# facebookresearch/vggsfm

Measured on AMD Instinct MI355X. Metric: BA LM-iterations/sec, higher is better.
Workload: dtype f64

## Files before the change

### vggsfm_amd/ba.py

```python
import copy
import ctypes
from dataclasses import dataclass
from typing import Optional

import math
import os

import numpy as np
import torch

from . import _lib
from .ba_options import LOSS_ID, TERMINATION, BundleAdjustmentOptions

MODEL_ID = {"SIMPLE_PINHOLE": 0, "SIMPLE_RADIAL": 1}
GROUP = 16
CHUNK = 1024
SUB = 32
MIN_CHUNK = 128
OVERLAP_FACTORIZATION = False
OVERLAP_MIN_OBS, OVERLAP_MIN_FRAMES = 1_000_000, 8 * GROUP
TILE_BATCHES = 3
CHOL_CUS = 32


# ... 664 lines not shown
                             camera_type, options, False, constant_points=constant, constant_pose_frames=[0],
                             filter_negative_depth=False)


def _c_options(options: BundleAdjustmentOptions, overlap=True):
    so = options.solver_options
    return _lib.BAOptions(so.max_num_iterations, so.max_num_consecutive_invalid_steps, int(so.jacobi_scaling),
                          so.function_tolerance, so.gradient_tolerance, so.parameter_tolerance,
                          so.initial_trust_region_radius, so.max_trust_region_radius, so.min_trust_region_radius,
                          so.min_lm_diagonal, so.max_lm_diagonal, so.min_relative_decrease,
                          CHOL_CUS if (overlap and OVERLAP_FACTORIZATION) else 0)


def _summary_dict(summ, log, n):
    its = [dict(iteration=l.iteration, cost=l.cost, cost_change=l.cost_change, gradient_max_norm=l.gradient_max_norm,
                step_norm=l.step_norm, relative_decrease=l.relative_decrease, radius=l.radius,
                successful=bool(l.successful)) for l in log[:n]]
    return dict(initial_cost=summ.initial_cost, final_cost=summ.final_cost, num_iterations=summ.num_iterations,
                num_successful_steps=summ.num_successful_steps, num_unsuccessful_steps=summ.num_unsuccessful_steps,
                termination=summ.termination, termination_str=TERMINATION.get(summ.termination, "?"),
                n_reduced=summ.n_reduced, iterations=its)


def solve(problem: DeviceProblem, options: Optional[BundleAdjustmentOptions] = None, workspace=None):
    L = _lib.lib()
    glue = _hook("VGGSFM_LEGACY_GLUE")
    if glue is not None:
        L.vgg_ba_set_tile_rhs(2 | (4 if glue == "1" else 0))
    options = options or BundleAdjustmentOptions()
    problem.refine_focal = options.refine_focal_length
    problem.refine_extra = options.refine_extra_params
    problem.loss = LOSS_ID[options.loss_function_type]
    problem.loss_scale = options.loss_function_scale
    cp = problem.c_struct()
    co = _c_options(options)
    nbytes = L.vgg_ba_workspace_bytes(ctypes.byref(cp), ctypes.byref(co))
    if workspace is None or workspace.numel() < nbytes:
        workspace = torch.empty(nbytes, dtype=torch.uint8, device=problem.pts.device)
    summ = _lib.BASummary()
    cap = options.solver_options.max_num_iterations + 2
    log = (_lib.BAIteration * cap)()
    _lib.check(L.vgg_ba_solve(ctypes.byref(cp), ctypes.byref(co), workspace, workspace.numel(), ctypes.byref(summ), log, cap,
                              _lib.stream_ptr()), "vgg_ba_solve")
    out = _summary_dict(summ, log, summ.num_log)
    if options.print_summary:
        print(f"Bundle adjustment report: residuals {problem.num_obs * 2}, parameters reduced {summ.n_reduced}, "
              f"iterations {summ.num_iterations}, cost {summ.initial_cost:.6g} -> {summ.final_cost:.6g}, "
              f"{out['termination_str']}")
    return out, workspace


# ... 73 lines not shown
```

### vggsfm_amd/csrc/ba.hip

```cpp
#include <mutex>
#include <type_traits>
#include <vector>

#include "camera_model.hpp"
#include "../../include/vggsfm_amd.h"

namespace vgg {

int cholesky_solve_enqueue(double* A, double* b, int n, double* inv_blocks, int32_t* device_fail, const int32_t* skip_flag,
                           hipStream_t st, const CholOverlap* overlap, int split_a, int split_b, const int32_t* first_blk,
                           bool flags_cleared);
int32_t* cholesky_dataflow_flags(double* ws, int n, size_t* count);
size_t cholesky_workspace_bytes(int n);
void dataflow_signal(int32_t* flag, hipStream_t st);

constexpr int kGroup = 16;
#ifndef VGG_OFFDIAG_OCC
#define VGG_OFFDIAG_OCC 3
#endif
#ifndef VGG_DIAG_OCC
#define VGG_DIAG_OCC 4
#endif
#ifndef VGG_DIAG_FULL_DEPTH
#define VGG_DIAG_FULL_DEPTH 2
// ... 17 lines not shown
#define VGG_PS_OCC 2
#endif
#ifndef VGG_CP_OCC_RHS
#define VGG_CP_OCC_RHS 2
#endif
#ifndef VGG_CP_OCC
#define VGG_CP_OCC 2
#endif
#ifndef VGG_ABLATE
#define VGG_ABLATE 0
#endif
constexpr int kSub = 32;
constexpr int kMaxWG = 2048;
constexpr int kCamSplitMax = 16;
constexpr int kCamNV = 48;
constexpr int kPackPad = 1024;

struct Ctl {
  double radius, decrease_factor, x_cost, initial_cost, gmax_cams, gmax, cand_cost, mcc, step_norm, rel;
  int32_t iteration, done, termination, need_lin, scale_ready, invalid_streak, num_succ, num_unsucc;
  int32_t linear_fail, accept, rank, world, grad_logged;
  int32_t step_arrivals;
  int32_t merged_glue_launches, merged_step_sums;
};

struct Dims {
  int C, P, O, NI, model, kd, only_k, shared, BDp, n_red, kdsh, loss;
  double loss_scale;
};

constexpr int kYc = 12;
static inline size_t y_slot_doubles(const Dims& d) { return (d.shared || d.kd == 0) ? (size_t)kYc : (size_t)d.BDp * 3; }

struct Ws {
  Ctl* ctl;
  vgg_ba_iteration* log;
  double *cand_q, *cand_t, *cand_intr, *cand_pts;
  double *scale_c, *scale_p, *colsq_c, *dsq_c, *dy;
  uint8_t* active;
  double* lin;
  double *U, *g, *costc;
  double* sys;
  double *S, *rhs;
  double* S2;
  double* gmax_pts;
  double* stepsum;
// ... 19 lines not shown
  int tile_rhs;
  double* lin_cand;
  double *U_cand, *g_cand, *cost_cand;
  size_t lin_count, sys_count, total_bytes;
};

static inline size_t align_up(size_t x, size_t a) { return (x + a - 1) / a * a; }


static Dims make_dims(const vgg_ba_problem* pb) {
  Dims d;
  d.C = pb->num_cams; d.P = pb->num_pts; d.O = pb->num_obs; d.NI = pb->num_intr; d.model = pb->camera_model;
  const int rf = pb->refine_focal ? 1 : 0, rk = (pb->refine_extra && pb->camera_model == kSimpleRadial) ? 1 : 0;
  d.kd = rf + rk;
  d.only_k = (!rf && rk) ? 1 : 0;
  d.shared = (pb->num_intr == 1) ? 1 : 0;
  d.BDp = 6 + d.kd;
  d.n_red = 6 * d.C + d.kd * d.NI;
  d.kdsh = d.shared ? d.kd : 0;
  d.loss = pb->loss; d.loss_scale = pb->loss_scale;
  return d;
}

struct Tuning { int lpp, longt, cam_wgs, point_wgs, tile_rhs, legacy_glue; };
static Tuning g_tuning = {0, -1, 0, 0, 2, 0};

static Ws carve(const Dims& d, int max_iters, int num_chunks, int num_segments, void* base) {
  Ws w;
  size_t off = 0;
  auto take = [&](size_t bytes) { size_t o = off; off = align_up(off + bytes, 256); return (char*)base + o; };
  w.ctl = (Ctl*)take(sizeof(Ctl));
  w.log = (vgg_ba_iteration*)take(sizeof(vgg_ba_iteration) * (size_t)(max_iters + 2));
  w.cand_q = (double*)take(8ull * 4 * d.C); w.cand_t = (double*)take(8ull * 3 * d.C);
  w.cand_intr = (double*)take(8ull * 4 * d.NI); w.cand_pts = (double*)take(8ull * 3 * d.P);
  w.scale_c = (double*)take(8ull * d.n_red); w.scale_p = (double*)take(8ull * 3 * d.P);
  w.colsq_c = (double*)take(8ull * d.n_red); w.dsq_c = (double*)take(8ull * d.n_red);
  w.dy = (double*)take(8ull * d.n_red);
  w.active = (uint8_t*)take(d.n_red);
  w.lin_count = (size_t)d.C * d.BDp * d.BDp + (size_t)d.C * d.BDp + d.C;
  w.lin = (double*)take(8ull * w.lin_count);
  w.U = w.lin; w.g = w.U + (size_t)d.C * d.BDp * d.BDp; w.costc = w.g + (size_t)d.C * d.BDp;
  w.sys_count = (size_t)d.n_red * d.n_red + d.n_red;
  w.sys = (double*)take(8ull * w.sys_count);
  w.S = w.sys; w.rhs = w.S + (size_t)d.n_red * d.n_red;
  w.S2 = (double*)take(8ull * (size_t)d.n_red * d.n_red);
  w.packed_count = (size_t)d.n_red * (d.n_red + 1) / 2 + d.n_red;
  w.packed = (double*)take(8ull * (w.packed_count + 2 * kPackPad));
  w.pk_mine = (double*)take(8ull * (w.packed_count + 2));
// ... 126 lines not shown
  }
  return rho[0];
}

__device__ __forceinline__ double loss_rho0(const Dims& d, double s) {
  double rho[3];
  loss_eval(d.loss, d.loss_scale, s, rho);
  return rho[0];
}

template <int NV>
__device__ __forceinline__ void block_sum(double* v, double* lds , double* out ) {
  const int wave = threadIdx.x >> 6, lane = threadIdx.x & 63;
#pragma unroll
  for (int i = 0; i < NV; ++i) {
    const double s = wave_sum(v[i]);
    if (lane == 0) lds[wave * NV + i] = s;
  }
  __syncthreads();
  if (threadIdx.x < NV) out[threadIdx.x] = lds[threadIdx.x] + lds[NV + threadIdx.x] + lds[2 * NV + threadIdx.x] + lds[3 * NV + threadIdx.x];
  __syncthreads();
}

__global__ void init_kernel(DevProblem pb, Ws w, vgg_ba_options opt, int rank, int world) {
  const Dims& d = pb.d;
  const int j = blockIdx.x * blockDim.x + threadIdx.x;
  if (j == 0) {
    Ctl c;
    memset(&c, 0, sizeof(c));
    c.radius = opt.initial_trust_region_radius; c.decrease_factor = 2.0; c.need_lin = 1; c.rank = rank; c.world = world;
    *w.ctl = c;
    w.gmax_pts[0] = 0; for (int i = 0; i < 4; ++i) w.stepsum[i] = 0;
  }
  if (j < d.n_red) {
    bool act;
    if (j < 6 * d.C) {
      const int c = j / 6, k = j - 6 * c;
      const unsigned f = pb.cam_const ? pb.cam_const[c] : 0u;
      act = (pb.col_ptr[c + 1] > pb.col_ptr[c]) || world > 1;
      if (f & 1u) act = false;
      if (k >= 3 && (f & (2u << (k - 3)))) act = false;
    } else {
      const int a = (j - 6 * d.C) / d.kd;
      act = !(pb.intr_const && pb.intr_const[a]);
      if (!d.shared && world == 1 && !(pb.col_ptr[a + 1] > pb.col_ptr[a])) act = false;
    }
// ... 91 lines not shown
#pragma unroll
        for (int k = i; k < BD; ++k) acc[u++] += F[i] * F[k] + F[BD + i] * F[BD + k];
#pragma unroll
      for (int i = 0; i < BD; ++i) acc[NU + i] += F[i] * r[0] + F[BD + i] * r[1];
      acc[NU + BD] += rho0;
    } else {
      double R0[1 + KD], R1[1 + KD];
      R0[0] = r[0] - (E[0] * h0 + E[1] * h1v + E[2] * h2);
      R1[0] = r[1] - (E[3] * h0 + E[4] * h1v + E[5] * h2);
#pragma unroll
      for (int m = 0; m < KD; ++m) {
        if (m < kdsh) {
          const double* M = Mc + 3 * m;
          R0[1 + m] = -(E[0] * M[0] + E[1] * M[1] + E[2] * M[2]);
          R1[1 + m] = -(E[3] * M[0] + E[4] * M[1] + E[5] * M[2]);
        } else { R0[1 + m] = 0; R1[1 + m] = 0; }
      }
#pragma unroll
      for (int i = 0; i < BD; ++i)
#pragma unroll
        for (int m = 0; m < 1 + KD; ++m) acc[i * (1 + KD) + m] += F[i] * R0[m] + F[BD + i] * R1[m];
    }
  }
  block_sum<NV>(acc, red, tot);
  static_assert(NV <= kCamNV, "cam_split row");
  if (threadIdx.x < NV) w.cam_split[((size_t)c * kCamSplitMax + blockIdx.y) * kCamNV + threadIdx.x] = tot[threadIdx.x];
}

template <bool BYPASS>
__device__ __forceinline__ void reduce_step_body(const Ws& w, int nparts, int C, double (*red)[256]) {
  auto ld = [](const double* p) -> double {
    return BYPASS ? __hip_atomic_load(p, __ATOMIC_RELAXED, __HIP_MEMORY_SCOPE_AGENT) : *p;
  };
  double s[4] = {0, 0, 0, 0};
  for (int i = threadIdx.x; i < C; i += 256) s[0] += ld(w.cost_cand + i);
  for (int i = threadIdx.x; i < nparts; i += 256)
    for (int k = 1; k < 4; ++k) s[k] += ld(w.part_F + 4 * i + k);
  for (int k = 0; k < 4; ++k) red[k][threadIdx.x] = s[k];
  __syncthreads();
  for (int st = 128; st > 0; st >>= 1) {
    if (threadIdx.x < st) for (int k = 0; k < 4; ++k) red[k][threadIdx.x] += red[k][threadIdx.x + st];
    __syncthreads();
  }
  if (threadIdx.x < 4) w.stepsum[threadIdx.x] = red[threadIdx.x][0];
}

template <int KD, int MODE>
// ... 1394 lines not shown
  for (; ch + 1 < c1; ch += 2) { s0 += src[(size_t)ch * R * R]; s1 += src[(size_t)(ch + 1) * R * R]; }
  if (ch < c1) s0 += src[(size_t)ch * R * R];
  const int hi = ri > cj ? ri : cj, lo = ri > cj ? cj : ri;
  double v = -(s0 + s1);
  if constexpr (BD == 6) {
    const double mi = w.active[ri] ? w.scale_c[ri] : 0.0, mj = w.active[cj] ? w.scale_c[cj] : 0.0;
    v *= mi * mj;
  }
  if (gI == gJ && a == b) {
    const double* U = w.U + (size_t)ca * UBD * UBD;
    double t = 0.0;
    if (global_terms) t = w.scale_c[ri] * w.scale_c[cj] * U[i * UBD + j];
    if (ri == cj) {
      const double dsq = lm_damping(U[i * UBD + i], w.scale_c[ri], radius, opt);
      w.dsq_c[ri] = dsq;
      if (global_terms) t += dsq;
    }
    v = v + t;
  }
  w.S[(size_t)hi * n + lo] = v;
}

template <int KD>
__global__ void cam_update_kernel(DevProblem pb, Ws w) {
  if (w.ctl->done) return;
  const Dims& d = pb.d;
  const int c = blockIdx.x * blockDim.x + threadIdx.x;
  if (c > d.C) return;
  double step = 0, xn = 0;
  if (c < d.C) {
    double dl[6];
    for (int k = 0; k < 6; ++k) {
      const int j = 6 * c + k;
      const double dyv = w.active[j] ? w.scale_c[j] * w.rhs[j] : 0.0;
      w.dy[j] = dyv;
      dl[k] = -dyv;
    }
    double qn[4];
    quat_plus(pb.cam_q + 4 * c, dl, qn);
    const bool pose_var = !(pb.cam_const && (pb.cam_const[c] & 1u));
    for (int k = 0; k < 4; ++k) { w.cand_q[4 * c + k] = qn[k]; const double df = qn[k] - pb.cam_q[4 * c + k]; step += df * df; if (pose_var) xn += pb.cam_q[4 * c + k] * pb.cam_q[4 * c + k]; }
    for (int k = 0; k < 3; ++k) { const double tn = pb.cam_t[3 * c + k] + dl[3 + k]; w.cand_t[3 * c + k] = tn; step += dl[3 + k] * dl[3 + k]; if (pose_var) xn += pb.cam_t[3 * c + k] * pb.cam_t[3 * c + k]; }
  }
  const int a = d.shared ? ((c == d.C) ? 0 : -1) : ((c < d.C) ? c : -1);
  if (a >= 0) {
    double in4[4];
    for (int k = 0; k < 4; ++k) in4[k] = pb.intr[4 * a + k];
    for (int k = 0; k < KD; ++k) {
      const int j = 6 * d.C + KD * a + k;
      const double dyv = w.active[j] ? w.scale_c[j] * w.rhs[j] : 0.0;
      w.dy[j] = dyv;
      const int slot = (KD == 2) ? (k == 0 ? 0 : 3) : (d.only_k ? 3 : 0);
      in4[slot] -= dyv;
      step += dyv * dyv;
    }
    const bool intr_var = KD > 0 && !(pb.intr_const && pb.intr_const[a]);
    const int np = (d.model == kSimpleRadial) ? 4 : 3;
    for (int k = 0; k < 4; ++k) { w.cand_intr[4 * a + k] = in4[k]; if (intr_var && k < np) xn += pb.intr[4 * a + k] * pb.intr[4 * a + k]; }
  }
  w.cam_part[3 * c] = step;
  w.cam_part[3 * c + 1] = xn;
  w.cam_part[3 * c + 2] = 0.0;
}

template <int KD, bool LDSCAM, int LPP, bool LONGT = false>
__global__ __launch_bounds__(256, VGG_PS_OCC) void point_step_kernel(DevProblem pb, Ws w) {
  constexpr int BD = 6 + KD;
  __shared__ double red[4][3];
  extern __shared__ double cam_cache[];
  if (w.ctl->done) return;
  const Dims& d = pb.d;
  constexpr int PPW = 64 / LPP;
  const int wave = threadIdx.x >> 6, lane = threadIdx.x & 63;
  const int sub = lane / LPP, sl = lane % LPP;
  const int nw = gridDim.x * 4 * PPW;
  double s_mcc = 0, s_step = 0, s_xn = 0;
  const double* lq = cam_cache;
  const double* lt = lq + 9 * d.C;
  const double* ldy = lt + 3 * d.C;
  const double* lfl = ldy + 6 * d.C;
  if (LDSCAM) {
    double* cc = cam_cache;
    for (int i = threadIdx.x; i < d.C; i += 256) {
      quat_to_R(pb.cam_q + 4 * i, cc + 9 * i);
      cc[18 * d.C + i] = pb.cam_const ? (double)pb.cam_const[i] : 0.0;
    }
    for (int i = threadIdx.x; i < 3 * d.C; i += 256) cc[9 * d.C + i] = pb.cam_t[i];
    for (int i = threadIdx.x; i < 6 * d.C; i += 256) cc[(ldy - cam_cache) + i] = w.dy[i];
    __syncthreads();
  }
  (void)lfl;
  int p = (blockIdx.x * 4 + wave) * PPW + sub;
  constexpr int NPF = LONGT ? 4 : 2;
  int n_o0 = 0, n_o1 = 0;
  ObsPf<NPF> n_pf;
  double n_X0 = 0, n_X1 = 0, n_X2 = 0;
  int n_ptc = 0;
  int m_o0 = 0, m_o1 = 0;
  double m_X0 = 0, m_X1 = 0, m_X2 = 0;
  int m_ptc = 0;
  if (p < d.P) {
    n_o0 = pb.row_ptr[p]; n_o1 = pb.row_ptr[p + 1];
    n_X0 = pb.pts[3 * p]; n_X1 = pb.pts[3 * p + 1]; n_X2 = pb.pts[3 * p + 2];
    n_ptc = pb.pt_const ? (int)pb.pt_const[p] : 0;
    n_pf.template load<false>(pb.obs_cam, pb.obs_uv, pb.obs_slot, n_o0, n_o1, LPP, sl);
    if (p + nw < d.P) {
      const int pm = p + nw;
      m_o0 = pb.row_ptr[pm]; m_o1 = pb.row_ptr[pm + 1];
      m_X0 = pb.pts[3 * pm]; m_X1 = pb.pts[3 * pm + 1]; m_X2 = pb.pts[3 * pm + 2];
      m_ptc = pb.pt_const ? (int)pb.pt_const[pm] : 0;
    }
  }
  for (; p < d.P; p += nw) {
    const int o0 = n_o0, o1 = n_o1;
    const double X[3] = {n_X0, n_X1, n_X2};
    const bool pt_c = n_ptc != 0;
    const ObsPf<NPF> f_pf = n_pf;
    {
      n_o0 = m_o0; n_o1 = m_o1; n_X0 = m_X0; n_X1 = m_X1; n_X2 = m_X2; n_ptc = m_ptc;
      if (p + nw < d.P) n_pf.template load<false>(pb.obs_cam, pb.obs_uv, pb.obs_slot, n_o0, n_o1, LPP, sl);
      const int pm = p + 2 * nw;
      if (pm < d.P) {
        m_o0 = pb.row_ptr[pm]; m_o1 = pb.row_ptr[pm + 1];
        m_X0 = pb.pts[3 * pm]; m_X1 = pb.pts[3 * pm + 1]; m_X2 = pb.pts[3 * pm + 2];
        m_ptc = pb.pt_const ? (int)pb.pt_const[pm] : 0;
      }
    }
    double t3[3] = {0, 0, 0};
    const double* Gp = w.G + 6 * (size_t)p;
    const double G00 = Gp[0], G01 = Gp[1], G02 = Gp[2], G11 = Gp[3], G12 = Gp[4], G22 = Gp[5];
    const double hs0 = w.hs[3 * (size_t)p], hs1 = w.hs[3 * (size_t)p + 1], hs2 = w.hs[3 * (size_t)p + 2];
    const double pd0 = w.pdamp[3 * (size_t)p], pd1 = w.pdamp[3 * (size_t)p + 1], pd2 = w.pdamp[3 * (size_t)p + 2];
    auto evaluated = [&](int pass, int o) __attribute__((always_inline)) {
      const int c = f_pf.cam(pass, pb.obs_cam, o);
      const float2 uv = f_pf.uv(pass, pb.obs_uv, o);
      const int a = d.shared ? 0 : c;
      double r[2], F[2 * BD], E[6];
      if (LDSCAM)
        eval_full<KD>(d, lq + 9 * c, lt + 3 * c, pb.intr + 4 * a, X, uv, (unsigned)lfl[c],
                      pb.intr_const ? pb.intr_const[a] != 0 : false, pt_c, r, F, E);
      else
        eval_full<KD>(d, CamR(pb.cam_q + 4 * c).R, pb.cam_t + 3 * c, pb.intr + 4 * a, X, uv,
                      pb.cam_const ? pb.cam_const[c] : 0u, pb.intr_const ? pb.intr_const[a] != 0 : false, pt_c, r, F, E);
      double fy0 = 0, fy1 = 0;
#pragma unroll
      for (int k = 0; k < 6; ++k) { const double v = LDSCAM ? ldy[6 * c + k] : w.dy[6 * c + k]; fy0 += F[k] * v; fy1 += F[BD + k] * v; }
#pragma unroll
      for (int k = 0; k < KD; ++k) { const double v = w.dy[6 * d.C + KD * a + k]; fy0 += F[6 + k] * v; fy1 += F[BD + 6 + k] * v; }
      t3[0] += E[0] * fy0 + E[3] * fy1; t3[1] += E[1] * fy0 + E[4] * fy1; t3[2] += E[2] * fy0 + E[5] * fy1;
      s_mcc += fy0 * (r[0] - 0.5 * fy0) + fy1 * (r[1] - 0.5 * fy1);
    };
    for (int o = o0 + sl; o < o1; o += LPP) evaluated((o - o0) / LPP, o);
#pragma unroll
    for (int i = 0; i < 3; ++i) t3[i] = group_sum<LPP>(t3[i]);
    const double u0 = G00 * t3[0], u1 = G01 * t3[0] + G11 * t3[1], u2 = G02 * t3[0] + G12 * t3[1] + G22 * t3[2];
    double ys[3];
    ys[0] = hs0 - (G00 * u0 + G01 * u1 + G02 * u2);
    ys[1] = hs1 - (G11 * u1 + G12 * u2);
    ys[2] = hs2 - (G22 * u2);
    if (sl == 0) {
      w.cand_pts[3 * (size_t)p] = X[0] - ys[0]; w.cand_pts[3 * (size_t)p + 1] = X[1] - ys[1]; w.cand_pts[3 * (size_t)p + 2] = X[2] - ys[2];
      s_step += ys[0] * ys[0] + ys[1] * ys[1] + ys[2] * ys[2];
      if (!pt_c) s_xn += X[0] * X[0] + X[1] * X[1] + X[2] * X[2];
      if (G22 != 0.0) {
        const double z2 = ys[2] / G22, z1 = (ys[1] - G12 * z2) / G11, z0 = (ys[0] - G01 * z1 - G02 * z2) / G00;
        s_mcc += 0.5 * (z0 * z0 + z1 * z1 + z2 * z2) + 0.5 * (pd0 * ys[0] * ys[0] + pd1 * ys[1] * ys[1] + pd2 * ys[2] * ys[2]);
      }
    }
  }
  s_mcc = wave_sum(s_mcc); s_step = wave_sum(s_step); s_xn = wave_sum(s_xn);
  if (lane == 0) { red[wave][0] = s_mcc; red[wave][1] = s_step; red[wave][2] = s_xn; }
// ... 430 lines not shown
    (void)hipEventRecord(oc->ready, L.st);
    (void)hipStreamWaitEvent(oc->st_rest, oc->ready, 0);
    (void)hipStreamWaitEvent(oc->st_chol, oc->ready, 0);
    launch_schur_batches<KD>(L, 1, L.num_batches, oc->st_rest, L.w.S2, L.w.batch_flags);
    CholOverlap ov;
    ov.dev_flags = L.w.batch_flags + 1;
    ov.S2 = L.w.S2;
    ov.first_col = 6 * kGroup * L.batches[6 * 1 + 5];
    ov.num_waits = L.num_batches - 1;
    for (int b = 1; b < L.num_batches; ++b) ov.wait_col[b - 1] = 6 * kGroup * L.batches[6 * b + 5];
    {
      ProfScope ps(kProfCholesky, oc->st_chol);
      rc = cholesky_solve_enqueue(L.w.S, L.w.rhs, d.n_red, L.w.chol_inv, &L.w.ctl->linear_fail, &L.w.ctl->done, oc->st_chol, &ov,
                                  L.chol_split_a, L.chol_split_b, L.chol_first_blk, true);
    }
    (void)hipEventRecord(oc->chol_done, oc->st_chol);
    (void)hipStreamWaitEvent(L.st, oc->chol_done, 0);
  } else {
    ProfScope ps(kProfCholesky, L.st);
    rc = cholesky_solve_enqueue(L.w.S, L.w.rhs, d.n_red, L.w.chol_inv, &L.w.ctl->linear_fail, &L.w.ctl->done, L.st, nullptr,
                                L.chol_split_a, L.chol_split_b, L.chol_first_blk, true);
  }
  if (rc != VGG_OK) return rc;
  cam_update_kernel<KD><<<div_up(d.C + 1, 64), 64, 0, L.st>>>(L.dp, L.w);
  {
    ProfScope ps(kProfPointStep, L.st);
    const size_t cam_lds = sizeof(double) * 19 * (size_t)d.C;
    auto launch = [&](auto lpp) {
      constexpr int LPP = decltype(lpp)::value;
      const bool longt = long_tracks(LPP, L.d.P, L.d.O);
      if (longt && LPP <= 32) {
        if (cam_lds <= 64 * 1024) point_step_kernel<KD, true, LPP, (LPP <= 32)><<<L.wgB, 256, cam_lds, L.st>>>(L.dp, L.w);
        else point_step_kernel<KD, false, LPP, (LPP <= 32)><<<L.wgB, 256, 0, L.st>>>(L.dp, L.w);
      } else if (cam_lds <= 64 * 1024) point_step_kernel<KD, true, LPP><<<L.wgB, 256, cam_lds, L.st>>>(L.dp, L.w);
      else point_step_kernel<KD, false, LPP><<<L.wgB, 256, 0, L.st>>>(L.dp, L.w);
    };
    if (L.lpp == 8) launch(std::integral_constant<int, 8>{});
    else if (L.lpp == 16) launch(std::integral_constant<int, 16>{});
    else if (L.lpp == 32) launch(std::integral_constant<int, 32>{});
    else launch(std::integral_constant<int, 64>{});
  }
  {
    ProfScope ps(kProfLinearize, L.st);
    DevProblem dc = L.dp;
    dc.cam_q = L.w.cand_q; dc.cam_t = L.w.cand_t; dc.intr = L.w.cand_intr; dc.pts = L.w.cand_pts;
    Ws wc = L.w;
    wc.U = L.w.U_cand; wc.g = L.w.g_cand; wc.costc = L.w.cost_cand;
    launch_linearize<KD>(L, dc, wc, g_tuning.legacy_glue ? 0 : L.wgB);
  }
  if (g_tuning.legacy_glue) reduce_step_kernel<<<1, 256, 0, L.st>>>(L.w, L.wgB, d.C);
  return VGG_OK;
}

static void phase_update(const Launch& L) {
  const Dims& d = L.d;
  control_kernel<<<1, 64, 0, L.st>>>(L.w, L.opt, d.C);
  size_t nmax = (size_t)3 * d.P;
  if ((size_t)4 * d.C > nmax) nmax = (size_t)4 * d.C;
  if ((size_t)4 * d.NI > nmax) nmax = (size_t)4 * d.NI;
  if (L.w.lin_count > nmax) nmax = L.w.lin_count;
  commit_kernel<<<div_up((long)nmax, 256), 256, 0, L.st>>>(L.w, L.cam_q, L.cam_t, L.intr, L.pts, d.C, d.NI, d.P);
}

// ... 93 lines not shown
    if (hipMemcpyAsync(log, L.w.log, sizeof(vgg_ba_iteration) * ncopy, hipMemcpyDeviceToHost, L.st) != hipSuccess) return VGG_ERR_HIP;
  }
  if (hipStreamSynchronize(L.st) != hipSuccess) return VGG_ERR_HIP;
  if (summary) {
    summary->initial_cost = h.initial_cost; summary->final_cost = h.x_cost;
    summary->num_iterations = h.iteration; summary->num_successful_steps = h.num_succ;
    summary->num_unsuccessful_steps = h.num_unsucc; summary->termination = h.termination;
    summary->n_reduced = L.d.n_red;
    summary->num_log = (h.iteration + 1 < ncopy) ? h.iteration + 1 : ncopy;
  }
  return VGG_OK;
}

}

using namespace vgg;

extern "C" {

int vgg_ba_tuning(int lanes_per_point, int long_tracks, int cam_workgroups, int point_workgroups) {
  if (!(lanes_per_point == 0 || lanes_per_point == 8 || lanes_per_point == 16 || lanes_per_point == 32 || lanes_per_point == 64))
    return VGG_ERR_INVALID_ARGUMENT;
  vgg::g_tuning = vgg::Tuning{lanes_per_point, long_tracks < 0 ? -1 : (long_tracks ? 1 : 0), cam_workgroups > 0 ? cam_workgroups : 0,
                              point_workgroups > 0 ? point_workgroups : 0, vgg::g_tuning.tile_rhs, vgg::g_tuning.legacy_glue};
  return VGG_OK;
}

int vgg_ba_set_tile_rhs(int enable) {
  const bool known = enable >= 0 && enable <= 7 && (enable & 3) <= 2;
  vgg::g_tuning.tile_rhs = known ? (enable & 3) : 1;
  vgg::g_tuning.legacy_glue = (known && (enable & 4)) ? 1 : 0;
  return VGG_OK;
}

int vgg_ba_profile(int enable, int max_launches_per_kernel) {
  for (int k = 0; k < kProfCount; ++k) {
    for (int i = 0; i < g_prof.cap; ++i) { (void)hipEventDestroy(g_prof.start[k][i]); (void)hipEventDestroy(g_prof.stop[k][i]); }
    delete[] g_prof.start[k]; delete[] g_prof.stop[k];
    g_prof.start[k] = g_prof.stop[k] = nullptr; g_prof.n[k] = 0;
  }
  g_prof.cap = 0; g_prof.on = false;
  if (!enable) return VGG_OK;
  if (max_launches_per_kernel <= 0) return VGG_ERR_INVALID_ARGUMENT;
  for (int k = 0; k < kProfCount; ++k) {
    g_prof.start[k] = new hipEvent_t[max_launches_per_kernel];
    g_prof.stop[k] = new hipEvent_t[max_launches_per_kernel];
    for (int i = 0; i < max_launches_per_kernel; ++i) {
      VGG_HIP_CHECK(hipEventCreate(&g_prof.start[k][i]));
      VGG_HIP_CHECK(hipEventCreate(&g_prof.stop[k][i]));
    }
  }
  g_prof.cap = max_launches_per_kernel; g_prof.on = true;
  return VGG_OK;
}
// ... 132 lines not shown
```

### vggsfm_amd/csrc/camera_model.hpp

```cpp
#pragma once
#include "common.hpp"

namespace vgg {

enum : int { kPinhole = 0, kSimpleRadial = 1 };
enum : int { kLossTrivial = 0, kLossCauchy = 1, kLossHuber = 2, kLossSoftL1 = 3 };

struct Pose {
  double q[4];
  double t[3];
};

__device__ __forceinline__ void quat_rotate(const double* q, const double* v, double* out) {
  double ux = q[1] * v[2] - q[2] * v[1], uy = q[2] * v[0] - q[0] * v[2], uz = q[0] * v[1] - q[1] * v[0];
  ux += ux; uy += uy; uz += uz;
  out[0] = v[0] + q[3] * ux + (q[1] * uz - q[2] * uy);
  out[1] = v[1] + q[3] * uy + (q[2] * ux - q[0] * uz);
  out[2] = v[2] + q[3] * uz + (q[0] * uy - q[1] * ux);
}

__device__ __forceinline__ void quat_to_R(const double* q, double* R) {
  const double x = q[0], y = q[1], z = q[2], w = q[3];
  const double tx = 2 * x, ty = 2 * y, tz = 2 * z;
  const double twx = tx * w, twy = ty * w, twz = tz * w, txx = tx * x, txy = ty * x, txz = tz * x;
  const double tyy = ty * y, tyz = tz * y, tzz = tz * z;
  R[0] = 1 - (tyy + tzz); R[1] = txy - twz; R[2] = txz + twy;
  R[3] = txy + twz; R[4] = 1 - (txx + tzz); R[5] = tyz - twx;
  R[6] = txz - twy; R[7] = tyz + twx; R[8] = 1 - (txx + tyy);
}

__device__ __forceinline__ void quat_plus(const double* x, const double* d, double* out) {
  const double n = sqrt(d[0] * d[0] + d[1] * d[1] + d[2] * d[2]);
  if (n == 0.0) { out[0] = x[0]; out[1] = x[1]; out[2] = x[2]; out[3] = x[3]; return; }
  const double s = sin(n) / n;
  const double qx = s * d[0], qy = s * d[1], qz = s * d[2], qw = cos(n);
  out[3] = qw * x[3] - qx * x[0] - qy * x[1] - qz * x[2];
  out[0] = qw * x[0] + qx * x[3] + qy * x[2] - qz * x[1];
  out[1] = qw * x[1] - qx * x[2] + qy * x[3] + qz * x[0];
  out[2] = qw * x[2] + qx * x[1] - qy * x[0] + qz * x[3];
}

__device__ __forceinline__ void obs_residual(int model, const double* q, const double* t, const double* intr,
                                             const double* X, double u_obs, double v_obs, double* r) {
  double a[3];
  quat_rotate(q, X, a);
  const double Y0 = a[0] + t[0], Y1 = a[1] + t[1], Y2 = a[2] + t[2];
  const double k = (model == kSimpleRadial) ? intr[3] : 0.0;
  const double iz = 1.0 / Y2;
  const double u = Y0 * iz, v = Y1 * iz;
  const double d = 1.0 + k * (u * u + v * v);
  r[0] = intr[0] * (u * d) + intr[1] - u_obs;
  r[1] = intr[0] * (v * d) + intr[2] - v_obs;
}

__device__ __forceinline__ void obs_eval(int model, const double* q, const double* t, const double* intr,
                                         const double* X, double u_obs, double v_obs, double* r, double* Jp,
                                         double* Ji, double* Jx) {
  double a[3];
  quat_rotate(q, X, a);
  const double Y0 = a[0] + t[0], Y1 = a[1] + t[1], Y2 = a[2] + t[2];
  const double f = intr[0];
  const double k = (model == kSimpleRadial) ? intr[3] : 0.0;
// ... 48 lines not shown
  const double k = (model == kSimpleRadial) ? intr[3] : 0.0;
  const double iz = 1.0 / Y2;
  const double u = Y0 * iz, v = Y1 * iz;
  const double r2 = u * u + v * v;
  const double d = 1.0 + k * r2;
  r[0] = f * (u * d) + intr[1] - u_obs;
  r[1] = f * (v * d) + intr[2] - v_obs;
  const double xu = f * (d + 2 * k * u * u), xv = f * (2 * k * u * v), yv = f * (d + 2 * k * v * v);
  double JY[6];
  JY[0] = xu * iz; JY[1] = xv * iz; JY[2] = -(xu * u + xv * v) * iz;
  JY[3] = xv * iz; JY[4] = yv * iz; JY[5] = -(xv * u + yv * v) * iz;
#pragma unroll
  for (int row = 0; row < 2; ++row) {
    const double* j = JY + 3 * row;
    Jp[row * 6 + 0] = 2.0 * (j[2] * a[1] - j[1] * a[2]);
    Jp[row * 6 + 1] = 2.0 * (j[0] * a[2] - j[2] * a[0]);
    Jp[row * 6 + 2] = 2.0 * (j[1] * a[0] - j[0] * a[1]);
    Jp[row * 6 + 3] = j[0]; Jp[row * 6 + 4] = j[1]; Jp[row * 6 + 5] = j[2];
#pragma unroll
    for (int c = 0; c < 3; ++c) Jx[row * 3 + c] = j[0] * R[c] + j[1] * R[3 + c] + j[2] * R[6 + c];
  }
  Ji[0] = u * d; Ji[1] = f * r2 * u;
  Ji[2] = v * d; Ji[3] = f * r2 * v;
}

__device__ __forceinline__ void loss_eval(int loss, double a, double s, double* rho) {
  const double b = a * a;
  if (loss == kLossCauchy) {
    const double sum = 1.0 + s / b, inv = 1.0 / sum;
    rho[0] = b * log(sum); rho[1] = fmax(inv, 2.2250738585072014e-308); rho[2] = -(1.0 / b) * (inv * inv);
  } else if (loss == kLossHuber) {
    if (s > b) { const double r = sqrt(s); rho[0] = 2 * a * r - b; rho[1] = fmax(a / r, 2.2250738585072014e-308); rho[2] = -rho[1] / (2 * s); }
    else { rho[0] = s; rho[1] = 1; rho[2] = 0; }
  } else if (loss == kLossSoftL1) {
    const double sum = 1.0 + s / b, tmp = sqrt(sum);
    rho[0] = 2 * b * (tmp - 1); rho[1] = fmax(1 / tmp, 2.2250738585072014e-308); rho[2] = -1 / (2 * b * tmp * sum);
  } else {
    rho[0] = s; rho[1] = 1; rho[2] = 0;
  }
}

struct Corrector {
  double sqrt_rho1, residual_scaling, alpha_sq_norm;
  __device__ __forceinline__ Corrector(double sq_norm, const double* rho) {
    sqrt_rho1 = sqrt(rho[1]);
    if (sq_norm == 0.0 || rho[2] <= 0.0) { residual_scaling = sqrt_rho1; alpha_sq_norm = 0.0; return; }
// ... 23 lines not shown
```

### vggsfm_amd/dist.py

```python
import ctypes

import torch

from . import _lib
from . import ba as BA
from .ba_options import LOSS_ID, BundleAdjustmentOptions


def partition_points(obs_per_point, world_size):
    counts = obs_per_point.to(torch.int64)
    P = counts.shape[0]
    csum = torch.cumsum(counts, 0)
    total = int(csum[-1].item()) if P > 0 else 0
    bounds = [0]
    for r in range(1, world_size):
        target = total * r / world_size
        idx = int(torch.searchsorted(csum, torch.tensor(target, dtype=csum.dtype, device=csum.device)).item())
        bounds.append(max(bounds[-1], min(idx, P)))
    bounds.append(P)
    return torch.tensor(bounds, dtype=torch.long)


def shard_slice(tracks, masks, points3d, rank, world_size):
    b = partition_points(masks.sum(0), world_size)
# ... 190 lines not shown
        off4 = self.bufs[4].data_ptr() - self.ws.data_ptr()
        assert world_size * (chunk + 1) <= self.bufs[6].numel(), "one-piece exchange: buffer 6 too small for world_size"
        self._padded = self.ws[off4:off4 + 8 * world_size * chunk].view(torch.float64)
        self._mine = self.bufs[5][:chunk + 1]
        self._gathered = self.bufs[6][:world_size * (chunk + 1)]
        self._in_place = isinstance(collectives, Collectives) and collectives.scatter
        want_split = SPLIT_EXCHANGE if split_exchange is None else bool(split_exchange)
        self._split = False
        if want_split and (self._in_place or split_exchange == "emulated"):
            if self.L.vgg_ba_phase(*self._abi, 12, _lib.stream_ptr()) == 0:
                W = max(world_size, 1)
                a = _lib.reduce_buffer(*self._abi, 7)[1]
                ca, cb = -(-a // W), -(-(M - a) // W)
                off5 = self.bufs[5].data_ptr() - self.ws.data_ptr()
                assert off4 + 8 * W * (ca + cb) <= off5, "split exchange: buffer 4 region overruns buffer 5"
                assert W * ca + W * (cb + 1) <= self.bufs[6].numel(), "split exchange: buffer 6 region overruns its carve"
                b4 = self.ws[off4:off4 + 8 * W * (ca + cb)].view(torch.float64)
                self._padded_a, self._padded_b = b4[:W * ca], b4[W * ca:]
                self._mine_a, self._mine_b = self.bufs[5][:ca], self.bufs[5][ca:ca + cb + 1]
                self._gathered_a, self._gathered_b = self.bufs[6][:W * ca], self.bufs[6][W * ca:W * ca + W * (cb + 1)]
                self._split = True

    def begin(self):
        _lib.check(self.L.vgg_ba_begin(*self._abi, self.nbytes, self.rank, self.world, _lib.stream_ptr()), "vgg_ba_begin")

    def _phase(self, i):
        _lib.check(self.L.vgg_ba_phase(*self._abi, i, _lib.stream_ptr()), "vgg_ba_phase")

    def iteration(self):
        co = self.coll
        self._phase(0)
        if co:
            co.sum_(self.bufs[0])
        if co and self._split:
            self._phase(7)
            self._phase(8)
            ha = co.system_scatter_begin(self._padded_a, self._mine_a, self._gathered_a, rides=0)
            self._phase(9)
            self._phase(10)
            hb = co.system_scatter_begin(self._padded_b, self._mine_b, self._gathered_b, rides=1)
            co.system_scatter_end(ha)
            co.system_scatter_end(hb)
            self._phase(11)
            self._phase(2)
            co.sum_(self.bufs[3])
            self._phase(3)
# ... 38 lines not shown
```

Baseline: 705.9.

## Fuse camera update into point-step kernel and compute step directly without full Jacobian

```diff
diff --git a/vggsfm_amd/ba.py b/vggsfm_amd/ba.py
--- a/vggsfm_amd/ba.py
+++ b/vggsfm_amd/ba.py
@@ -710,11 +710,15 @@
                 n_reduced=summ.n_reduced, iterations=its)
 
 
+def apply_launch_hooks(L):
+    glue, step = _hook("VGGSFM_LEGACY_GLUE"), _hook("VGGSFM_LEGACY_STEP")
+    if glue is not None or step is not None:
+        L.vgg_ba_set_tile_rhs(2 | (4 if glue == "1" else 0) | (8 if step == "1" else 0))
+
+
 def solve(problem: DeviceProblem, options: Optional[BundleAdjustmentOptions] = None, workspace=None):
     L = _lib.lib()
-    glue = _hook("VGGSFM_LEGACY_GLUE")
-    if glue is not None:
-        L.vgg_ba_set_tile_rhs(2 | (4 if glue == "1" else 0))
+    apply_launch_hooks(L)
     options = options or BundleAdjustmentOptions()
     problem.refine_focal = options.refine_focal_length
     problem.refine_extra = options.refine_extra_params
diff --git a/vggsfm_amd/csrc/ba.hip b/vggsfm_amd/csrc/ba.hip
--- a/vggsfm_amd/csrc/ba.hip
+++ b/vggsfm_amd/csrc/ba.hip
@@ -63,6 +63,7 @@
   int32_t linear_fail, accept, rank, world, grad_logged;
   int32_t step_arrivals;
   int32_t merged_glue_launches, merged_step_sums;
+  int32_t fused_step_prologues;
 };
 
 struct Dims {
@@ -128,8 +129,8 @@
   return d;
 }
 
-struct Tuning { int lpp, longt, cam_wgs, point_wgs, tile_rhs, legacy_glue; };
-static Tuning g_tuning = {0, -1, 0, 0, 2, 0};
+struct Tuning { int lpp, longt, cam_wgs, point_wgs, tile_rhs, legacy_glue, legacy_step; };
+static Tuning g_tuning = {0, -1, 0, 0, 2, 0, 0};
 
 static Ws carve(const Dims& d, int max_iters, int num_chunks, int num_segments, void* base) {
   Ws w;
@@ -302,6 +303,34 @@
   __syncthreads();
 }
 
+template <int N, int OFF>
+__device__ __forceinline__ void wave_reduce_scatter(double* v, int lane, int n, int base, double* dst) {
+  if constexpr (OFF == 0) {
+    static_assert(N == 1, "64 lanes hold at most 64 values");
+    if (n > 0) dst[base] = v[0];
+  } else {
+    constexpr int H = (N + 1) / 2;
+    const bool hi = (lane & OFF) != 0;
+    double k[H];
+#pragma unroll
+    for (int i = 0; i < H; ++i) {
+      const double up = (H + i < N) ? v[H + i] : 0.0;
+      const double send = hi ? v[i] : up, keep = hi ? up : v[i];
+      k[i] = keep + __shfl_xor(send, OFF, 64);
+    }
+    wave_reduce_scatter<H, OFF / 2>(k, lane, hi ? max(n - H, 0) : min(n, H), base + (hi ? H : 0), dst);
+  }
+}
+template <int NV>
+__device__ __forceinline__ void block_sum_scatter(double* v, double* lds , double* out ) {
+  static_assert(NV <= 64, "one value per lane at the end");
+  const int wave = threadIdx.x >> 6, lane = threadIdx.x & 63;
+  wave_reduce_scatter<NV, 32>(v, lane, NV, 0, lds + wave * NV);
+  __syncthreads();
+  if (threadIdx.x < NV) out[threadIdx.x] = lds[threadIdx.x] + lds[NV + threadIdx.x] + lds[2 * NV + threadIdx.x] + lds[3 * NV + threadIdx.x];
+  __syncthreads();
+}
+
 __global__ void init_kernel(DevProblem pb, Ws w, vgg_ba_options opt, int rank, int world) {
   const Dims& d = pb.d;
   const int j = blockIdx.x * blockDim.x + threadIdx.x;
@@ -439,7 +468,8 @@
         for (int m = 0; m < 1 + KD; ++m) acc[i * (1 + KD) + m] += F[i] * R0[m] + F[BD + i] * R1[m];
     }
   }
-  block_sum<NV>(acc, red, tot);
+  if (MODE == 0) block_sum_scatter<NV>(acc, red, tot);
+  else block_sum<NV>(acc, red, tot);
   static_assert(NV <= kCamNV, "cam_split row");
   if (threadIdx.x < NV) w.cam_split[((size_t)c * kCamSplitMax + blockIdx.y) * kCamNV + threadIdx.x] = tot[threadIdx.x];
 }
@@ -1880,49 +1910,81 @@
 }
 
 template <int KD>
-__global__ void cam_update_kernel(DevProblem pb, Ws w) {
-  if (w.ctl->done) return;
+__device__ __forceinline__ void cam_update_body(const DevProblem& pb, const Ws& w, int c, bool cam_mcc) {
+  constexpr int BD = 6 + KD;
   const Dims& d = pb.d;
-  const int c = blockIdx.x * blockDim.x + threadIdx.x;
-  if (c > d.C) return;
-  double step = 0, xn = 0;
+  double step = 0, xn = 0, mcc = 0;
   if (c < d.C) {
-    double dl[6];
+    double dl[6], dyc[BD];
+#pragma unroll
     for (int k = 0; k < 6; ++k) {
       const int j = 6 * c + k;
       const double dyv = w.active[j] ? w.scale_c[j] * w.rhs[j] : 0.0;
       w.dy[j] = dyv;
+      dyc[k] = dyv;
       dl[k] = -dyv;
     }
     double qn[4];
-    quat_plus(pb.cam_q + 4 * c, dl, qn);
+    quat_plus_select(pb.cam_q + 4 * c, dl, qn);
     const bool pose_var = !(pb.cam_const && (pb.cam_const[c] & 1u));
+#pragma unroll
     for (int k = 0; k < 4; ++k) { w.cand_q[4 * c + k] = qn[k]; const double df = qn[k] - pb.cam_q[4 * c + k]; step += df * df; if (pose_var) xn += pb.cam_q[4 * c + k] * pb.cam_q[4 * c + k]; }
+#pragma unroll
     for (int k = 0; k < 3; ++k) { const double tn = pb.cam_t[3 * c + k] + dl[3 + k]; w.cand_t[3 * c + k] = tn; step += dl[3 + k] * dl[3 + k]; if (pose_var) xn += pb.cam_t[3 * c + k] * pb.cam_t[3 * c + k]; }
+    if (cam_mcc) {
+#pragma unroll
+      for (int k = 0; k < KD; ++k) {
+        const int j = 6 * d.C + KD * (d.shared ? 0 : c) + k;
+        dyc[6 + k] = w.active[j] ? w.scale_c[j] * w.rhs[j] : 0.0;
+      }
+      const double* U = w.U + (size_t)c * BD * BD;
+      const double* g = w.g + (size_t)c * BD;
+      double lin = 0, quad = 0;
+#pragma unroll
+      for (int i = 0; i < BD; ++i) {
+        double ud = 0;
+#pragma unroll
+        for (int k = 0; k < BD; ++k) ud += U[i * BD + k] * dyc[k];
+        lin += dyc[i] * g[i];
+        quad += dyc[i] * ud;
+      }
+      mcc = lin - 0.5 * quad;
+    }
   }
   const int a = d.shared ? ((c == d.C) ? 0 : -1) : ((c < d.C) ? c : -1);
   if (a >= 0) {
     double in4[4];
+#pragma unroll
     for (int k = 0; k < 4; ++k) in4[k] = pb.intr[4 * a + k];
+#pragma unroll
     for (int k = 0; k < KD; ++k) {
       const int j = 6 * d.C + KD * a + k;
       const double dyv = w.active[j] ? w.scale_c[j] * w.rhs[j] : 0.0;
       w.dy[j] = dyv;
-      const int slot = (KD == 2) ? (k == 0 ? 0 : 3) : (d.only_k ? 3 : 0);
-      in4[slot] -= dyv;
+      const bool extra = (KD == 2) ? (k == 1) : (d.only_k != 0);
+      if (extra) in4[3] -= dyv; else in4[0] -= dyv;
       step += dyv * dyv;
     }
     const bool intr_var = KD > 0 && !(pb.intr_const && pb.intr_const[a]);
     const int np = (d.model == kSimpleRadial) ? 4 : 3;
+#pragma unroll
     for (int k = 0; k < 4; ++k) { w.cand_intr[4 * a + k] = in4[k]; if (intr_var && k < np) xn += pb.intr[4 * a + k] * pb.intr[4 * a + k]; }
   }
   w.cam_part[3 * c] = step;
   w.cam_part[3 * c + 1] = xn;
-  w.cam_part[3 * c + 2] = 0.0;
-}
-
-template <int KD, bool LDSCAM, int LPP, bool LONGT = false>
-__global__ __launch_bounds__(256, VGG_PS_OCC) void point_step_kernel(DevProblem pb, Ws w) {
+  w.cam_part[3 * c + 2] = mcc;
+}
+
+template <int KD>
+__global__ void cam_update_kernel(DevProblem pb, Ws w, int cam_mcc) {
+  if (w.ctl->done) return;
+  const int c = blockIdx.x * blockDim.x + threadIdx.x;
+  if (c > pb.d.C) return;
+  cam_update_body<KD>(pb, w, c, cam_mcc != 0);
+}
+
+template <int KD, bool LDSCAM, int LPP, bool LONGT = false, bool DIR = true>
+__global__ __launch_bounds__(256, VGG_PS_OCC) void point_step_kernel(DevProblem pb, Ws w, int fused) {
   constexpr int BD = 6 + KD;
   __shared__ double red[4][3];
   extern __shared__ double cam_cache[];
@@ -1936,18 +1998,31 @@
   const double* lq = cam_cache;
   const double* lt = lq + 9 * d.C;
   const double* ldy = lt + 3 * d.C;
-  const double* lfl = ldy + 6 * d.C;
+  const double* ldi = ldy + 6 * d.C;
+  const uint8_t* lfl = reinterpret_cast<const uint8_t*>(ldi + KD * d.NI);
   if (LDSCAM) {
     double* cc = cam_cache;
     for (int i = threadIdx.x; i < d.C; i += 256) {
       quat_to_R(pb.cam_q + 4 * i, cc + 9 * i);
-      cc[18 * d.C + i] = pb.cam_const ? (double)pb.cam_const[i] : 0.0;
+      if (!DIR) reinterpret_cast<uint8_t*>(cc + 12 * d.C + d.n_red)[i] = pb.cam_const ? pb.cam_const[i] : (uint8_t)0;
     }
     for (int i = threadIdx.x; i < 3 * d.C; i += 256) cc[9 * d.C + i] = pb.cam_t[i];
-    for (int i = threadIdx.x; i < 6 * d.C; i += 256) cc[(ldy - cam_cache) + i] = w.dy[i];
+    if (fused) {
+#pragma unroll 4
+      for (int i = threadIdx.x; i < d.n_red; i += 256) cc[12 * d.C + i] = w.active[i] ? w.scale_c[i] * w.rhs[i] : 0.0;
+      const int nbody = min((int)gridDim.x, (d.C + 256) / 256);
+      const int jb = (int)gridDim.x - 1 - (int)blockIdx.x;
+      if (jb < nbody) {
+        for (int c = jb * 256 + threadIdx.x; c <= d.C; c += 256 * nbody) cam_update_body<KD>(pb, w, c, DIR);
+        if (jb == 0 && threadIdx.x == 0) w.ctl->fused_step_prologues += 1;
+      }
+    } else {
+#pragma unroll 4
+      for (int i = threadIdx.x; i < d.n_red; i += 256) cc[12 * d.C + i] = w.dy[i];
+    }
     __syncthreads();
   }
-  (void)lfl;
+  (void)lfl; (void)ldi;
   int p = (blockIdx.x * 4 + wave) * PPW + sub;
   constexpr int NPF = LONGT ? 4 : 2;
   int n_o0 = 0, n_o1 = 0;
@@ -1993,6 +2068,40 @@
       const int c = f_pf.cam(pass, pb.obs_cam, o);
       const float2 uv = f_pf.uv(pass, pb.obs_uv, o);
       const int a = d.shared ? 0 : c;
+      if constexpr (DIR) {
+        double dyp[6], di[2] = {0.0, 0.0};
+#pragma unroll
+        for (int k = 0; k < 6; ++k) dyp[k] = LDSCAM ? ldy[6 * c + k] : w.dy[6 * c + k];
+#pragma unroll
+        for (int k = 0; k < KD; ++k) di[k] = LDSCAM ? ldi[KD * a + k] : w.dy[6 * d.C + KD * a + k];
+        const double df = (KD == 2 || (KD == 1 && !d.only_k)) ? di[0] : 0.0;
+        const double dk = (KD == 2) ? di[1] : ((KD == 1 && d.only_k) ? di[0] : 0.0);
+        double Rg[9];
+        const double* Rc = lq + 9 * c;
+        if (!LDSCAM) { quat_to_R(pb.cam_q + 4 * c, Rg); Rc = Rg; }
+        const ObsStep s = obs_step_R(d.model, Rc, LDSCAM ? lt + 3 * c : pb.cam_t + 3 * c, pb.intr + 4 * a, X, dyp, df, dk,
+                                     (double)uv.x, (double)uv.y);
+        double y[2] = {s.fy[0], s.fy[1]};
+        if (d.loss != kLossTrivial) {
+          const double sq = s.r[0] * s.r[0] + s.r[1] * s.r[1];
+          double rho[3];
+          loss_eval(d.loss, d.loss_scale, sq, rho);
+          const Corrector cor(sq, rho);
+#pragma unroll
+          for (int rep = 0; rep < 2; ++rep) {
+            const double rty = cor.alpha_sq_norm * (s.r[0] * y[0] + s.r[1] * y[1]);
+            y[0] = cor.sqrt_rho1 * (y[0] - s.r[0] * rty);
+            y[1] = cor.sqrt_rho1 * (y[1] - s.r[1] * rty);
+          }
+        }
+        double v3[3];
+        s.adjoint(y, v3);
+        if (!pt_c) {
+#pragma unroll
+          for (int k = 0; k < 3; ++k) t3[k] += Rc[k] * v3[0] + Rc[3 + k] * v3[1] + Rc[6 + k] * v3[2];
+        }
+        return;
+      }
       double r[2], F[2 * BD], E[6];
       if (LDSCAM)
         eval_full<KD>(d, lq + 9 * c, lt + 3 * c, pb.intr + 4 * a, X, uv, (unsigned)lfl[c],
@@ -2004,7 +2113,7 @@
 #pragma unroll
       for (int k = 0; k < 6; ++k) { const double v = LDSCAM ? ldy[6 * c + k] : w.dy[6 * c + k]; fy0 += F[k] * v; fy1 += F[BD + k] * v; }
 #pragma unroll
-      for (int k = 0; k < KD; ++k) { const double v = w.dy[6 * d.C + KD * a + k]; fy0 += F[6 + k] * v; fy1 += F[BD + 6 + k] * v; }
+      for (int k = 0; k < KD; ++k) { const double v = LDSCAM ? ldi[KD * a + k] : w.dy[6 * d.C + KD * a + k]; fy0 += F[6 + k] * v; fy1 += F[BD + 6 + k] * v; }
       t3[0] += E[0] * fy0 + E[3] * fy1; t3[1] += E[1] * fy0 + E[4] * fy1; t3[2] += E[2] * fy0 + E[5] * fy1;
       s_mcc += fy0 * (r[0] - 0.5 * fy0) + fy1 * (r[1] - 0.5 * fy1);
     };
@@ -2481,23 +2590,31 @@
                                 L.chol_split_a, L.chol_split_b, L.chol_first_blk, true);
   }
   if (rc != VGG_OK) return rc;
-  cam_update_kernel<KD><<<div_up(d.C + 1, 64), 64, 0, L.st>>>(L.dp, L.w);
+  const bool dir = !g_tuning.legacy_step;
+  const size_t cam_lds = sizeof(double) * (12 * (size_t)d.C + (size_t)d.n_red) + (dir ? 0 : align_up((size_t)d.C, 8));
+  const bool lds_cam = cam_lds <= 64 * 1024;
+  const int fused = (lds_cam && !g_tuning.legacy_glue) ? 1 : 0;
+  if (!fused) cam_update_kernel<KD><<<div_up(d.C + 1, 64), 64, 0, L.st>>>(L.dp, L.w, dir ? 1 : 0);
   {
     ProfScope ps(kProfPointStep, L.st);
-    const size_t cam_lds = sizeof(double) * 19 * (size_t)d.C;
-    auto launch = [&](auto lpp) {
+    auto launch = [&](auto lpp, auto dirc) {
       constexpr int LPP = decltype(lpp)::value;
+      constexpr bool DIR = decltype(dirc)::value;
       const bool longt = long_tracks(LPP, L.d.P, L.d.O);
       if (longt && LPP <= 32) {
-        if (cam_lds <= 64 * 1024) point_step_kernel<KD, true, LPP, (LPP <= 32)><<<L.wgB, 256, cam_lds, L.st>>>(L.dp, L.w);
-        else point_step_kernel<KD, false, LPP, (LPP <= 32)><<<L.wgB, 256, 0, L.st>>>(L.dp, L.w);
-      } else if (cam_lds <= 64 * 1024) point_step_kernel<KD, true, LPP><<<L.wgB, 256, cam_lds, L.st>>>(L.dp, L.w);
-      else point_step_kernel<KD, false, LPP><<<L.wgB, 256, 0, L.st>>>(L.dp, L.w);
+        if (lds_cam) point_step_kernel<KD, true, LPP, (LPP <= 32), DIR><<<L.wgB, 256, cam_lds, L.st>>>(L.dp, L.w, fused);
+        else point_step_kernel<KD, false, LPP, (LPP <= 32), DIR><<<L.wgB, 256, 0, L.st>>>(L.dp, L.w, 0);
+      } else if (lds_cam) point_step_kernel<KD, true, LPP, false, DIR><<<L.wgB, 256, cam_lds, L.st>>>(L.dp, L.w, fused);
+      else point_step_kernel<KD, false, LPP, false, DIR><<<L.wgB, 256, 0, L.st>>>(L.dp, L.w, 0);
     };
-    if (L.lpp == 8) launch(std::integral_constant<int, 8>{});
-    else if (L.lpp == 16) launch(std::integral_constant<int, 16>{});
-    else if (L.lpp == 32) launch(std::integral_constant<int, 32>{});
-    else launch(std::integral_constant<int, 64>{});
+    auto launch_lpp = [&](auto dirc) {
+      if (L.lpp == 8) launch(std::integral_constant<int, 8>{}, dirc);
+      else if (L.lpp == 16) launch(std::integral_constant<int, 16>{}, dirc);
+      else if (L.lpp == 32) launch(std::integral_constant<int, 32>{}, dirc);
+      else launch(std::integral_constant<int, 64>{}, dirc);
+    };
+    if (dir) launch_lpp(std::true_type{});
+    else launch_lpp(std::false_type{});
   }
   {
     ProfScope ps(kProfLinearize, L.st);
@@ -2637,14 +2754,16 @@
   if (!(lanes_per_point == 0 || lanes_per_point == 8 || lanes_per_point == 16 || lanes_per_point == 32 || lanes_per_point == 64))
     return VGG_ERR_INVALID_ARGUMENT;
   vgg::g_tuning = vgg::Tuning{lanes_per_point, long_tracks < 0 ? -1 : (long_tracks ? 1 : 0), cam_workgroups > 0 ? cam_workgroups : 0,
-                              point_workgroups > 0 ? point_workgroups : 0, vgg::g_tuning.tile_rhs, vgg::g_tuning.legacy_glue};
+                              point_workgroups > 0 ? point_workgroups : 0, vgg::g_tuning.tile_rhs, vgg::g_tuning.legacy_glue,
+                              vgg::g_tuning.legacy_step};
   return VGG_OK;
 }
 
 int vgg_ba_set_tile_rhs(int enable) {
-  const bool known = enable >= 0 && enable <= 7 && (enable & 3) <= 2;
+  const bool known = enable >= 0 && enable <= 15 && (enable & 3) <= 2;
   vgg::g_tuning.tile_rhs = known ? (enable & 3) : 1;
   vgg::g_tuning.legacy_glue = (known && (enable & 4)) ? 1 : 0;
+  vgg::g_tuning.legacy_step = (known && (enable & 8)) ? 1 : 0;
   return VGG_OK;
 }
 
diff --git a/vggsfm_amd/csrc/camera_model.hpp b/vggsfm_amd/csrc/camera_model.hpp
--- a/vggsfm_amd/csrc/camera_model.hpp
+++ b/vggsfm_amd/csrc/camera_model.hpp
@@ -38,6 +38,18 @@
   out[0] = qw * x[0] + qx * x[3] + qy * x[2] - qz * x[1];
   out[1] = qw * x[1] - qx * x[2] + qy * x[3] + qz * x[0];
   out[2] = qw * x[2] + qx * x[1] - qy * x[0] + qz * x[3];
+}
+
+__device__ __forceinline__ void quat_plus_select(const double* x, const double* d, double* out) {
+  const double n = sqrt(d[0] * d[0] + d[1] * d[1] + d[2] * d[2]);
+  const bool zero = n == 0.0;
+  const double s = sin(n) / n;
+  const double qx = s * d[0], qy = s * d[1], qz = s * d[2], qw = cos(n);
+  const double o3 = qw * x[3] - qx * x[0] - qy * x[1] - qz * x[2];
+  const double o0 = qw * x[0] + qx * x[3] + qy * x[2] - qz * x[1];
+  const double o1 = qw * x[1] - qx * x[2] + qy * x[3] + qz * x[0];
+  const double o2 = qw * x[2] + qx * x[1] - qy * x[0] + qz * x[3];
+  out[0] = zero ? x[0] : o0; out[1] = zero ? x[1] : o1; out[2] = zero ? x[2] : o2; out[3] = zero ? x[3] : o3;
 }
 
 __device__ __forceinline__ void obs_residual(int model, const double* q, const double* t, const double* intr,
@@ -132,6 +144,42 @@
   }
   Ji[0] = u * d; Ji[1] = f * r2 * u;
   Ji[2] = v * d; Ji[3] = f * r2 * v;
+}
+
+struct ObsStep {
+  double fy[2], r[2];
+  double iz, u, v, xu, xv, yv;
+  __device__ __forceinline__ void adjoint(const double* y, double* v3) const {
+    const double s0 = (xu * y[0] + xv * y[1]) * iz, s1 = (xv * y[0] + yv * y[1]) * iz;
+    v3[0] = s0; v3[1] = s1; v3[2] = -(u * s0 + v * s1);
+  }
+};
+__device__ __forceinline__ ObsStep obs_step_R(int model, const double* R, const double* t, const double* intr, const double* X,
+                                              const double* dpose, double df, double dk, double u_obs, double v_obs) {
+  ObsStep s;
+  double a[3];
+  a[0] = R[0] * X[0] + R[1] * X[1] + R[2] * X[2];
+  a[1] = R[3] * X[0] + R[4] * X[1] + R[5] * X[2];
+  a[2] = R[6] * X[0] + R[7] * X[1] + R[8] * X[2];
+  const double Y0 = a[0] + t[0], Y1 = a[1] + t[1], Y2 = a[2] + t[2];
+  const double f = intr[0];
+  const double k = (model == kSimpleRadial) ? intr[3] : 0.0;
+  const double iz = 1.0 / Y2;
+  const double u = Y0 * iz, v = Y1 * iz;
+  const double r2 = u * u + v * v;
+  const double d = 1.0 + k * r2;
+  s.r[0] = f * (u * d) + intr[1] - u_obs;
+  s.r[1] = f * (v * d) + intr[2] - v_obs;
+  s.xu = f * (d + 2 * k * u * u); s.xv = f * (2 * k * u * v); s.yv = f * (d + 2 * k * v * v);
+  const double w0 = 2.0 * (dpose[1] * a[2] - dpose[2] * a[1]) + dpose[3];
+  const double w1 = 2.0 * (dpose[2] * a[0] - dpose[0] * a[2]) + dpose[4];
+  const double w2 = 2.0 * (dpose[0] * a[1] - dpose[1] * a[0]) + dpose[5];
+  const double p0 = (w0 - u * w2) * iz, p1 = (w1 - v * w2) * iz;
+  const double gi = d * df + (f * r2) * dk;
+  s.fy[0] = s.xu * p0 + s.xv * p1 + u * gi;
+  s.fy[1] = s.xv * p0 + s.yv * p1 + v * gi;
+  s.iz = iz; s.u = u; s.v = v;
+  return s;
 }
 
 __device__ __forceinline__ void loss_eval(int loss, double a, double s, double* rho) {
diff --git a/vggsfm_amd/dist.py b/vggsfm_amd/dist.py
--- a/vggsfm_amd/dist.py
+++ b/vggsfm_amd/dist.py
@@ -236,6 +236,7 @@
                 self._split = True
 
     def begin(self):
+        BA.apply_launch_hooks(self.L)
         _lib.check(self.L.vgg_ba_begin(*self._abi, self.nbytes, self.rank, self.world, _lib.stream_ptr()), "vgg_ba_begin")
 
     def _phase(self, i):
```

New measurement: 727.0 (median of 6 runs). +3.0%, better.
